# adaly/gridnext

Measured on AMD Instinct MI355X. Metric: spots/sec training throughput (multimodal f+g), higher is better.
Workload: dtype f32; 1 GPU; C4: multimodal f(DenseNet-121 @128px + count-MLP 2000 genes) + hex g on 78x64 Visium grids, 1 array (4992 spots) per GPU per step, f frozen/eval (tutorial mode), g trained with Adam, masked CE; spots_per_array=4992, parallelism=dp1

## Files before the change

### gridnext_amd/_lib.py

```python
import ctypes
import os

import torch

_HERE = os.path.dirname(os.path.abspath(__file__))
LIB_PATH = os.environ.get('GNX_LIB') or os.path.join(_HERE, 'libgridnext_hip.so')

_P, _I, _L, _F, _D = ctypes.c_void_p, ctypes.c_int, ctypes.c_long, ctypes.c_float, ctypes.c_double

SIGNATURES = {
    'gnx_hexconv_fwd': (_I, [_P, _P, _P, _P, _P, _I, _I, _I, _I, _I, _I, _P]),
    'gnx_hexconv_bwd_data': (_I, [_P, _P, _P, _P, _I, _I, _I, _I, _I, _I, _P]),
    'gnx_hexconv_bwd_weight_workspace': (_L, [_I, _I, _I, _I, _I]),
    'gnx_hexconv_bwd_weight': (_I, [_P, _P, _P, _P, _P, _P, _I, _I, _I, _I, _I, _I, _I, _P]),
    'gnx_hexconv_bwd_weight_batch': (_I, [_P, _I, _P]),
    'gnx_bn_workspace': (_L, [_L, _I]),
    'gnx_bn_train_stats': (_I, [_P, _L, _L, _I, _P, _P, _P, _P, _P, _F, _F, _P, _P, _P, _P, _P, _P]),
    'gnx_bn_train_stats_sync': (_I, [_P, _L, _L, _I, _P, _P, _P, _P, _P, _F, _F, _P, _P, _P, _P, _P, _P, _P]),
    'gnx_bn_train_stats_apply': (_I, [_P, _L, _L, _I, _P, _P, _P, _P, _P, _F, _F, _P, _P, _P, _P, _P, _L, _I, _P, _P]),
    'gnx_bn_sync_words': (_L, [_I]),
    'gnx_bn_train_stats_apply_sync': (_I, [_P, _L, _L, _I, _P, _P, _P, _P, _P, _F, _F, _P, _P, _P, _P, _P, _L, _I, _P, _P, _P]),
    'gnx_bn_relu_bwd_sync': (_I, [_P, _L, _P, _L, _P, _L, _L, _I, _P, _P, _P, _P, _P, _P, _I, _I, _I, _I, _P, _P, _P]),
    'gnx_bn_fold_eval': (_I, [_I, _P, _P, _P, _P, _F, _P, _P, _P, _P, _P]),
    'gnx_scale_shift_relu': (_I, [_P, _L, _P, _L, _L, _I, _P, _P, _I, _P]),
# ... 1 lines not shown
    'gnx_bnrelu_avgpool2': (_I, [_P, _L, _P, _L, _L, _I, _I, _P, _P, _P]),
    'gnx_bn_relu_bwd_pooled': (_I, [_P, _L, _P, _L, _P, _L, _L, _I, _I, _P, _P, _P, _P, _P, _P, _I, _P, _P]),
    'gnx_colsum': (_I, [_P, _L, _L, _I, _P, _I, _P, _P]),
    'gnx_masked_ce_workspace': (_L, [_L]),
    'gnx_masked_ce_fwd': (_I, [_P, _L, _P, _L, _I, _I, _F, _P, _P, _P, _P, _P]),
    'gnx_masked_ce_bwd': (_I, [_P, _L, _P, _L, _I, _I, _P, _P, _F, _P, _L, _P]),
    'gnx_meter_add': (_I, [_P, _P, _D, _P, _P, _D, _P]),
    'gnx_conv1x1_bnrelu': (_I, [_P, _L, _P, _P, _L, _L, _I, _I, _P, _P, _I, _I, _P]),
    'gnx_conv1x1_workspace': (_L, [_L, _I, _I]),
    'gnx_conv1x1_bnrelu_ws': (_I, [_P, _L, _P, _P, _L, _L, _I, _I, _P, _P, _P, _P]),
    'gnx_conv1x1_bnrelu_act': (_I, [_P, _L, _P, _P, _L, _L, _I, _I, _P, _P, _P, _P, _P]),
    'gnx_conv1x1_split_pack_halves': (_L, [_I]),
    'gnx_conv1x1_split_pack': (_I, [_P, _P, _I, _P]),
    'gnx_conv1x1_bnrelu_act_split': (_I, [_P, _L, _P, _P, _L, _L, _I, _P, _P, _P, _P, _P]),
    'gnx_conv3x3_split_pack_halves': (_L, []),
    'gnx_conv3x3_split_pack': (_I, [_P, _P, _P]),
    'gnx_conv3x3_split': (_I, [_P, _L, _P, _P, _L, _L, _I, _P]),
    'gnx_wgrad1x1_split_workspace': (_L, [_L, _I, _I]),
    'gnx_wgrad1x1_split': (_I, [_P, _L, _P, _L, _P, _P, _P, _P, _L, _I, _I, _I, _P]),
    'gnx_wgrad3x3_split_workspace': (_L, [_L]),
    'gnx_wgrad3x3_split': (_I, [_P, _L, _P, _L, _P, _P, _L, _I, _I, _P]),
    'gnx_conv1x1_dgrad_bn_workspace': (_L, [_L, _I]),
    'gnx_conv1x1_dgrad_bnrelu_bwd': (_I, [_P, _L, _P, _P, _L, _P, _L, _L, _I, _I, _P, _P, _P, _P, _P, _P, _I, _P, _P]),
    'gnx_conv1x1_dgrad_wgrad_workspace': (_L, [_L, _I]),
    'gnx_conv1x1_dgrad_wgrad_bnrelu_bwd': (_I, [_P, _L, _P, _P, _L, _P, _L, _L, _I, _P, _P, _P, _P, _P, _P, _P, _P, _I, _P]),
    'gnx_conv3x3_dgrad_bn_workspace': (_L, [_L, _I]),
    'gnx_conv3x3_dgrad_bnrelu_bwd': (_I, [_P, _L, _P, _P, _L, _P, _L, _L, _I, _I, _I, _P, _P, _P, _P, _P, _P, _I, _P, _P]),
    'gnx_conv1x1_fold_clamp': (_I, [_P, _P, _P, _P, _P, _P, _P, _P, _I, _I, _P]),
    'gnx_conv1x1_clamped_act': (_I, [_P, _L, _P, _P, _P, _L, _L, _I, _I, _P, _P, _P]),
    'gnx_repack_conv3x3': (_I, [_P, _P, _I, _I, _P]),
    'gnx_conv1x1_bnrelu_f16': (_I, [_P, _L, _P, _P, _L, _L, _I, _I, _P, _P, _I, _I, _P]),
    'gnx_conv3x3_bnrelu_f16': (_I, [_P, _L, _P, _P, _L, _L, _I, _I, _I, _P, _P, _P]),
    'gnx_conv1x1_bnrelu_f16_act16': (_I, [_P, _L, _P, _P, _L, _L, _I, _I, _P, _P, _P, _P, _P]),
    'gnx_conv3x3_f16_dma': (_I, [_P, _L, _P, _P, _L, _L, _I, _I, _I, _P]),
    'gnx_conv_stem_bnrelu_maxpool_h16': (_I, [_P, _P, _P, _L, _L, _I, _I, _I, _I, _I, _I, _I, _I, _P, _P, _P]),
    'gnx_conv_stem_bnrelu_maxpool_u8': (_I, [_P, _P, _P, _L, _L, _I, _I, _I, _I, _I, _I, _I, _I, _P, _P, _P, _I, _P]),
    'gnx_conv_stem_bnrelu_maxpool_f16mul': (_I, [_P, _I, _P, _P, _L, _L, _I, _I, _I, _I, _I, _I, _I, _I, _P, _P, _P, _P]),
    'gnx_u8_to_f32': (_I, [_P, _P, _L, _I, _I, _I, _P, _P]),
    'gnx_conv1x1_bnrelu_f16_h': (_I, [_P, _L, _P, _P, _L, _L, _I, _I, _P, _P, _P, _P, _I, _I, _P]),
    'gnx_conv1x1_bnrelu_h16': (_I, [_P, _L, _P, _P, _L, _L, _I, _I, _P, _P, _P, _P, _P]),
    'gnx_bnrelu_avgpool2_h16': (_I, [_P, _L, _P, _L, _L, _I, _I, _P, _P, _P]),
    'gnx_conv3x3_f16_dma_h': (_I, [_P, _L, _P, _P, _L, _L, _I, _I, _I, _P]),
    'gnx_bnrelu_avgpool_h16': (_I, [_P, _L, _P, _L, _L, _I, _I, _P, _P, _P]),
    'gnx_wgrad1x1_f16_workspace': (_L, [_L, _I, _I]),
    'gnx_wgrad1x1_f16': (_I, [_P, _L, _P, _L, _P, _P, _P, _P, _L, _I, _I, _P, _I, _P, _P]),
    'gnx_wgrad3x3_f16_workspace': (_L, [_L]),
    'gnx_wgrad3x3_f16': (_I, [_P, _L, _P, _P, _P, _L, _I, _P, _I, _P, _P]),
    'gnx_conv3x3_dgrad_bnrelu_bwd_f16_workspace': (_L, [_L]),
    'gnx_conv3x3_dgrad_bnrelu_bwd_f16': (_I, [_P, _L, _P, _P, _P, _L, _I, _P, _P, _P, _P, _P, _P, _P, _I, _P, _P]),
    'gnx_conv1x1_dgrad_bnrelu_bwd_f16_workspace': (_L, [_L, _I]),
    'gnx_conv1x1_dgrad_bnrelu_bwd_f16': (_I, [_P, _P, _P, _L, _P, _L, _L, _I, _P, _P, _P, _P, _P, _P, _P, _P, _I, _P, _P]),
    'gnx_conv1x1_dgrad_wgrad_f16_workspace': (_L, [_L, _I]),
    'gnx_conv1x1_dgrad_wgrad_bnrelu_bwd_f16': (_I, [_P, _P, _P, _L, _P, _L, _L, _I, _P, _P, _P, _P, _P, _P, _P, _P, _P, _I, _P, _P]),
    'gnx_tail_bwd_f16_workspace': (_L, [_L, _I]),
    'gnx_tail_bwd_f16': (_I, [_P, _L, _P, _L, _P, _L, _L, _I, _I, _P, _P, _P, _P, _P, _P, _P, _P, _I, _P, _P]),
    'gnx_trans_bwd_f16_workspace': (_L, [_L, _I, _I]),
    'gnx_trans_bwd_f16': (_I, [_P, _L, _P, _L, _P, _L, _L, _I, _I, _P, _P, _P, _P, _P, _P, _P, _P, _I, _P, _P]),
    'gnx_h16_cols_to_f32': (_I, [_P, _L, _P, _L, _L, _I, _P, _P, _P]),
    'gnx_stem_bwd_f16_workspace': (_L, [_L, _I]),
    'gnx_stem_bwd_f16': (_I, [_P, _P, _P, _P, _P, _P, _P, _L, _P, _P, _P, _P, _L, _I, _I, _P, _I, _P, _P]),
    'gnx_dense_layer_f16_pack': (_I, [_P, _P, _P, _P, _I, _P]),
    'gnx_dense_layer_f16': (_I, [_P, _L, _L, _I, _I, _P, _P, _P, _P, _P, _P, _P]),
    'gnx_dense_layer_f16_tape': (_I, [_P, _L, _L, _I, _I, _P, _P, _P, _P, _P, _P, _P, _L, _P]),
    'gnx_dense_layer_f16_set_form': (_I, [_I]),
    'gnx_dense_bwd_f16_pack': (_I, [_P, _P, _P, _P, _I, _P]),
    'gnx_wgrad3x3_f16_lb': (_I, [_P, _L, _P, _L, _L, _P, _P, _L, _I, _P, _I, _P, _P]),
    'gnx_conv3x3_dgrad_bnrelu_bwd_f16_lb': (_I, [_P, _L, _P, _P, _L, _L, _P, _L, _I, _P, _P, _P, _P, _P, _P, _P, _I, _P, _P]),
    'gnx_conv3x3_bwd_f16_workspace': (_L, [_L]),
    'gnx_conv3x3_bwd_f16_lb': (_I, [_P, _L, _P, _P, _L, _L, _P, _P, _L, _I, _P, _P, _P, _P, _P, _P, _P, _I, _P, _P]),
    'gnx_conv1x1_dgrad_wgrad_bnrelu_bwd_f16_lb': (_I, [_P, _P, _P, _L, _L, _P, _L, _L, _L, _I, _P, _P, _P, _P, _P, _P, _P, _P, _P, _I,
                                                       _P, _P]),
    'gnx_tail_bwd_f16_lb': (_I, [_P, _L, _P, _L, _L, _P, _L, _L, _L, _I, _I, _P, _P, _P, _P, _P, _P, _P, _P, _I, _P, _P]),
    'gnx_trans_bwd_f16_lb': (_I, [_P, _L, _L, _P, _L, _L, _P, _L, _L, _L, _I, _I, _P, _P, _P, _P, _P, _P, _P, _P, _I, _P, _P]),
    'gnx_conv_stem_bnrelu_maxpool_f16mul_cb': (_I, [_P, _I, _P, _P, _L, _L, _I, _I, _I, _I, _I, _I, _I, _I, _P, _P, _P, _P]),
    'gnx_conv1x1_bnrelu_h16_cb': (_I, [_P, _L, _P, _P, _L, _L, _I, _I, _P, _P, _P, _P, _P]),
    'gnx_bnrelu_avgpool2_h16_cb': (_I, [_P, _L, _P, _L, _L, _I, _I, _P, _P, _P]),
    'gnx_transition_f16_pack': (_I, [_P, _P, _I, _I, _P]),
    'gnx_transition_f16': (_I, [_P, _L, _L, _I, _I, _I, _P, _P, _P, _P, _L, _P]),
    'gnx_transition_f16_tape': (_I, [_P, _L, _L, _I, _I, _I, _P, _P, _P, _P, _L, _P, _L, _P]),
    'gnx_bnrelu_avgpool_h16_cb': (_I, [_P, _L, _P, _L, _L, _I, _I, _P, _P, _P]),
    'gnx_conv3x3_bnrelu': (_I, [_P, _L, _P, _P, _L, _L, _I, _I, _I, _P, _P, _P]),
    'gnx_winograd_conv3x3_weights': (_I, [_P, _P, _I, _I, _P]),
    'gnx_conv3x3_winograd': (_I, [_P, _L, _P, _P, _L, _L, _I, _I, _I, _P]),
    'gnx_conv_stem': (_I, [_P, _P, _P, _L, _L, _I, _I, _I, _I, _I, _I, _I, _I, _P]),
    'gnx_conv_stem_bnrelu_maxpool': (_I, [_P, _P, _P, _L, _L, _I, _I, _I, _I, _I, _I, _I, _I, _P, _P, _P]),
    'gnx_conv_stem_bnrelu_maxpool_argmax': (_I, [_P, _P, _P, _L, _P, _L, _I, _I, _I, _I, _I, _I, _I, _I, _P, _P, _P]),
    'gnx_bnrelu_maxpool': (_I, [_P, _L, _P, _L, _L, _I, _I, _I, _P, _P, _P]),
    'gnx_bnrelu_avgpool': (_I, [_P, _L, _P, _L, _L, _I, _I, _P, _P, _P]),
    'gnx_wgrad_workspace': (_L, [_L, _I, _I, _I]),
    'gnx_wgrad_bnrelu': (_I, [_P, _L, _P, _L, _P, _P, _P, _P, _L, _I, _I, _I, _I, _I, _I, _P]),
    'gnx_wgrad_bnrelu_batch': (_I, [_P, _I, _I, _P]),
    'gnx_transpose_weight': (_I, [_P, _P, _I, _I, _P]),
    'gnx_relayout_weights_batch': (_I, [_P, _I, _I, _P]),
    'gnx_repack_conv3x3_bwd': (_I, [_P, _P, _I, _I, _P]),
    'gnx_rows_broadcast': (_I, [_P, _L, _P, _L, _L, _I, _I, _F, _P]),
    'gnx_avgpool2_bwd': (_I, [_P, _L, _P, _L, _L, _I, _I, _P]),
    'gnx_maxpool_bwd': (_I, [_P, _L, _P, _L, _P, _L, _P, _L, _L, _I, _I, _I, _P, _P, _P]),
    'gnx_bnrelu_maxpool_argmax': (_I, [_P, _L, _P, _L, _P, _L, _I, _I, _I, _P, _P, _P]),
    'gnx_maxpool_bwd_argmax': (_I, [_P, _P, _L, _P, _L, _L, _I, _I, _I, _P]),
    'gnx_maxpool_bwd_argmax_bnrelu': (_I, [_P, _P, _L, _P, _L, _P, _P, _L, _L, _I, _I, _I, _P]),
    'gnx_conv0_wgrad_workspace': (_L, [_L, _I, _I, _I, _I, _I, _I, _I]),
    'gnx_conv0_wgrad': (_I, [_P, _P, _L, _P, _P, _L, _I, _I, _I, _I, _I, _I, _I, _I, _P]),
    'gnx_softmax_rows': (_I, [_P, _L, _L, _I, _P, _L, _P, _P]),
    'gnx_gemm_f32': (_I, [_P, _L, _I, _P, _L, _I, _P, _P, _L, _L, _L, _L, _I, _P]),
    'gnx_gemm_f32_workspace': (_L, [_L, _L, _L]),
    'gnx_gemm_f32_ws': (_I, [_P, _L, _I, _P, _L, _I, _P, _P, _L, _L, _L, _L, _I, _P, _P]),
}

_lib = None
_ERRORS = {-1: 'bad argument', -2: 'kernel launch failed', -3: 'unsupported shape'}
ERR_UNSUPPORTED = -3


class HipExtensionMissing(RuntimeError):
    pass


def lib():
    global _lib
    if _lib is None:
        if not os.path.exists(LIB_PATH):
            raise HipExtensionMissing(
                "gridnext_amd: %s not found. Build it with `python -c 'import __graft_entry__ as g; g.build()'` "
                "or `make -C gridnext_amd/csrc`. There is no CPU fallback." % LIB_PATH)
        handle = ctypes.CDLL(LIB_PATH)
        for name, (res, args) in SIGNATURES.items():
            fn = getattr(handle, name)
            fn.restype, fn.argtypes = res, args
        _lib = handle
    return _lib


def stream():
    return torch.cuda.current_stream().cuda_stream


def ptr(t, dtype=torch.float32):
    if t is None:
        return None
    if not t.is_cuda:
        raise RuntimeError("gridnext_amd kernels need tensors on a HIP device (got %s); there is no CPU path"
                           % t.device)
    if dtype is not None and t.dtype != dtype:
        raise TypeError("expected %s, got %s" % (dtype, t.dtype))
    return t.data_ptr()


def call(name, *args):
    rc = getattr(lib(), name)(*args)
    if rc != 0:
        raise RuntimeError("%s failed: %s (%d)" % (name, _ERRORS.get(rc, 'error'), rc))


def try_call(name, *args):
    rc = getattr(lib(), name)(*args)
    if rc == ERR_UNSUPPORTED:
        return False
    if rc != 0:
        raise RuntimeError("%s failed: %s (%d)" % (name, _ERRORS.get(rc, 'error'), rc))
    return True


def query(name, *args):
    return getattr(lib(), name)(*args)
```

### gridnext_amd/csrc/conv3x3.hip

```cpp
#include "fwd_common.h"

namespace {

constexpr int C3_BM = 128, C3_BN = 32;

__global__ __launch_bounds__(256) void conv3x3_kernel(const float* __restrict__ A, long lda,
                                                      const float* __restrict__ Wr, float* __restrict__ out, long ldc,
                                                      long M, int N, int K, int S, const float* __restrict__ scale,
                                                      const float* __restrict__ shift, int vecA, int vecW) {
    extern __shared__ __attribute__((aligned(16))) float lds[];
    const int strip = C3_BM + 2 * S + 2;
    float* As = lds;
    float* Bs = lds + strip * LDK;
    const int t = threadIdx.x, lane = t & 63, wave = t >> 6, h = lane >> 5, i = lane & 31;
    const long P0 = (long)blockIdx.x * C3_BM;
    const long base = P0 - S - 1;
    const int n0 = blockIdx.y * C3_BN;
    const bool has_act = scale != nullptr;

    const long P = P0 + 32 * wave + i;
    unsigned mask = 0;
    if (P < M) {
        const int rem = (int)(P % ((long)S * S));
        const int y = rem / S, x = rem - y * S;
// ... 586 lines not shown
            {
                const char* raw = lds + OFF_RAW + par * RAWB;
#pragma unroll
                for (int j = 0; j < NIT; ++j) {
                    const int it = t + 256 * j;
                    const int c = it / NVR, jp = it - c * NVR;
                    if (it < NVR * 4 && jp < NV) {
                        const int xin = (2 * jp) & (S - 1);
                        auto at = [&](int q) {
                            return raw + (q >> 4) * 1024 + c * 256 + (((q & 15) + ((q >> 4) & 1)) & 15) * 16;
                        };
                        const char* zr = lds + OFF_Z;
                        typedef float f2 __attribute__((ext_vector_type(2)));
                        struct F4 { f2 lo, hi; };
                        auto rd = [&](const char* p) { return *reinterpret_cast<const F4*>(p); };
                        const F4 d0 = rd(xin == 0 ? zr : at(2 * jp)), d1 = rd(at(2 * jp + 1)), d2 = rd(at(2 * jp + 2)),
                                 d3 = rd(xin + 2 == S ? zr : at(2 * jp + 3));
                        char* v = lds + OFF_V + (jp >> 4) * 1024 + c * 256 + (jp & 15) * 16;
                        *reinterpret_cast<F4*>(v) = F4{d0.lo - d2.lo, d0.hi - d2.hi};
                        *reinterpret_cast<F4*>(v + VB) = F4{d1.lo + d2.lo, d1.hi + d2.hi};
                        *reinterpret_cast<F4*>(v + 2 * VB) = F4{d2.lo - d1.lo, d2.hi - d1.hi};
                        *reinterpret_cast<F4*>(v + 3 * VB) = F4{d1.lo - d3.lo, d1.hi - d3.hi};
                    }
                }
            }
#endif
            asm volatile("s_waitcnt lgkmcnt(0)" ::: "memory");
            asm volatile("s_barrier" ::: "memory");
            const unsigned bU = fU + par * UB;
            auto rdA = [&](auto e_c) {
                constexpr int e = decltype(e_c)::value;
                return lds_read4<(e & 1) * 512>(bV[e >> 1]);
            };
            auto rdB = [&](auto e_c) {
                constexpr int e = decltype(e_c)::value;
                return lds_read4<(e >> 1) * 2048 + (e & 1) * 512>(bU);
            };
            f32x4 a = rdA(std::integral_constant<int, 0>{}), bq = rdB(std::integral_constant<int, 0>{});
            static_for<0, 24>([&](auto step_c) {
                constexpr int step = decltype(step_c)::value;
                constexpr int xi = (step >> 1) & 3;
                f32x4 na, nb;
                if constexpr (step < 23) {
                    na = rdA(std::integral_constant<int, step + 1>{});
                    nb = rdB(std::integral_constant<int, step + 1>{});
                    asm volatile("s_waitcnt lgkmcnt(2)" : "+v"(a), "+v"(bq));
                } else {
                    asm volatile("s_waitcnt lgkmcnt(0)" : "+v"(a), "+v"(bq));
                }
                acc[xi][0] = __builtin_amdgcn_mfma_f32_32x32x2f32(a[0], bq[0], acc[xi][0], 0, 0, 0);
                acc[xi][1] = __builtin_amdgcn_mfma_f32_32x32x2f32(a[1], bq[1], acc[xi][1], 0, 0, 0);
                acc[xi][0] = __builtin_amdgcn_mfma_f32_32x32x2f32(a[2], bq[2], acc[xi][0], 0, 0, 0);
                acc[xi][1] = __builtin_amdgcn_mfma_f32_32x32x2f32(a[3], bq[3], acc[xi][1], 0, 0, 0);
#if GNX_WINO_DBG != 2
                if constexpr (step < NSR + NSU) issue_slot(step_c, par ^ 1);
#endif
                if constexpr (step < 23) { a = na; bq = nb; }
            });
            advance_next();
        };
        for (int c2 = 0; c2 < nk2; ++c2) {
            do_chunk(std::integral_constant<int, 0>{});
            do_chunk(std::integral_constant<int, 1>{});
        }
        {
            const int left = M - tile * BM;
            const __amdgpu_buffer_rsrc_t ro = __builtin_amdgcn_make_buffer_rsrc(
                out + (long)tile * BM * ldc, 0, (left < BM ? left : BM) * ldc * 4, 0x00020000);
            const int vo = (2 * (32 * wave + 4 * h) * ldc + i) * 4;
#pragma unroll
            for (int e = 0; e < 16; ++e) {
                const float m0 = acc[0][0][e] + acc[0][1][e], m1 = acc[1][0][e] + acc[1][1][e];
                const float m2 = acc[2][0][e] + acc[2][1][e], m3 = acc[3][0][e] + acc[3][1][e];
                const int row = 2 * ((e & 3) + 8 * (e >> 2));
                __builtin_amdgcn_raw_buffer_store_b32(__float_as_uint((m0 + m1) + m2), ro, vo, row * ldc * 4, 0);
                __builtin_amdgcn_raw_buffer_store_b32(__float_as_uint((m1 - m2) - m3), ro, vo, (row + 1) * ldc * 4, 0);
            }
        }
        stored = true;
    }
    asm volatile("s_waitcnt vmcnt(0)" ::: "memory");
}

__global__ void winograd_weights_kernel(const float* __restrict__ w, float* __restrict__ wu, int N, int K) {
    const long idx = (long)blockIdx.x * blockDim.x + threadIdx.x;
    const long total = (long)3 * N * K;
    if (idx >= total) return;
    const int k = (int)(idx % K), n = (int)((idx / K) % N), dy = (int)(idx / ((long)K * N));
    const float* g = w + ((long)n * K + k) * 9 + dy * 3;
    const float g0 = g[0], g1 = g[1], g2 = g[2];
    const long nk = (long)N * K;
    float* u = wu + (long)dy * 4 * nk + (long)n * K + k;
    u[0] = g0;
    u[nk] = 0.5f * ((g0 + g2) + g1);
    u[2 * nk] = 0.5f * ((g0 + g2) - g1);
    u[3 * nk] = g2;
}

__global__ void repack3x3_kernel(const float* __restrict__ w, float* __restrict__ wr, int N, int K) {
    const long idx = (long)blockIdx.x * blockDim.x + threadIdx.x;
    const long total = (long)9 * N * K;
    if (idx >= total) return;
    const int k = (int)(idx % K), n = (int)((idx / K) % N), tap = (int)(idx / ((long)K * N));
    wr[idx] = w[((long)n * K + k) * 9 + tap];
}

}

GNX_EXPORT int gnx_repack_conv3x3(const float* w, float* wr, int N, int K, hipStream_t stream) {
    if (!w || !wr || N <= 0 || K <= 0) return GNX_ERR_BAD_ARG;
    repack3x3_kernel<<<gnx_cdiv(9L * N * K, 256), 256, 0, stream>>>(w, wr, N, K);
    return gnx_launch_status();
}

GNX_EXPORT int gnx_winograd_conv3x3_weights(const float* w, float* wu, int N, int K, hipStream_t stream) {
    if (!w || !wu || N <= 0 || K <= 0) return GNX_ERR_BAD_ARG;
    winograd_weights_kernel<<<gnx_cdiv(3L * N * K, 256), 256, 0, stream>>>(w, wu, N, K);
    return gnx_launch_status();
}

GNX_EXPORT int gnx_conv3x3_winograd(const float* A, long lda, const float* Wu, float* out, long ldc, long M, int N, int K,
                                    int S, hipStream_t stream) {
    if (!A || !Wu || !out || M < 0 || N <= 0 || K <= 0 || S <= 0 || lda < K || ldc < N || (M % ((long)S * S)) != 0)
        return GNX_ERR_BAD_ARG;
    if (N != 32 || (K & 31) != 0 || !al16(A) || !al16(Wu) || lda % 4 != 0 ||
        M * (lda > ldc ? lda : ldc) >= (1L << 31))
        return GNX_ERR_UNSUPPORTED;
    if (M == 0) return GNX_OK;
    const long wgs = (M + 255) / 256 > 256 ? 256 : (M + 255) / 256;
#define GNX_WINO(SS)                                                                                        \
    conv3x3_wino_kernel<SS><<<(int)wgs, 256, 0, stream>>>(A, (int)lda, Wu, out, (int)ldc, (int)M, K);        \
    return gnx_launch_status()
    switch (S) {
        case 4: GNX_WINO(4);
        case 8: GNX_WINO(8);
        case 16: GNX_WINO(16);
        case 32: GNX_WINO(32);
        case 64: GNX_WINO(64);
        default: return GNX_ERR_UNSUPPORTED;
    }
#undef GNX_WINO
}

GNX_EXPORT long gnx_conv3x3_dgrad_bn_workspace(long M, int N) { return 256L * 8 * 2 * N; }

GNX_EXPORT int gnx_conv3x3_dgrad_bnrelu_bwd(const float* dY, long lddy, const float* Wb, const float* A_act, long lda,
                                            float* dX, long lddx, long M, int N, int K, int S, const float* scale,
                                            const float* shift, const float* mean, const float* invstd, float* dgamma,
                                            float* dbeta, int accumulate, float* workspace, hipStream_t stream) {
    if (!dY || !Wb || !A_act || !dX || !scale || !shift || !mean || !invstd || !workspace || M < 0 || N <= 0 || K <= 0 ||
        S <= 0 || lddy < K || lda < N || lddx < N || (M % ((long)S * S)) != 0)
        return GNX_ERR_BAD_ARG;
    if (K != 32 || N != 128 || (M % C3_BM) != 0 || !al16(dY) || !al16(Wb) || lddy % 4 != 0 ||
        M * (lddy > lddx ? (lddy > lda ? lddy : lda) : (lddx > lda ? lddx : lda)) >= (1L << 31))
        return GNX_ERR_UNSUPPORTED;
    if (M == 0) return GNX_OK;
    C3BnAdj bn = {A_act, (int)lda, scale, shift, mean, invstd, workspace};
    int nblk = 0;
#define GNX_DMAA(SS)                                                                                              \
    do {                                                                                                          \
        if constexpr (SS <= 32) {                                                                                 \
            if (M % 256 == 0 && M / 256 >= 1024) {                                                                \
                nblk = 256 * 8;                                                                                   \
                conv3x3_dma_kernel<SS, 8, 32, true, false, false, true><<<256, 512, 0, stream>>>(                 \
                    dY, (int)lddy, Wb, dX, (int)lddx, (int)M, K, N, bn);                                          \
                break;                                                                                            \
            }                                                                                                     \
        }                                                                                                         \
        const long wgs = M / 128 > 256 ? 256 : M / 128;                                                           \
        nblk = (int)wgs * 4;                                                                                      \
        conv3x3_dma_kernel<SS, 4, 32, true, false, false, true><<<(int)wgs, 256, 0, stream>>>(                    \
            dY, (int)lddy, Wb, dX, (int)lddx, (int)M, K, N, bn);                                                  \
    } while (0)
    switch (S) {
        case 4: GNX_DMAA(4); break;
        case 8: GNX_DMAA(8); break;
        case 16: GNX_DMAA(16); break;
        case 32: GNX_DMAA(32); break;
        case 64: GNX_DMAA(64); break;
        default: return GNX_ERR_UNSUPPORTED;
    }
#undef GNX_DMAA
    if (dgamma || dbeta)
        c3_adj_reduce_kernel<<<gnx_cdiv(2 * N, 64), 64 * C3_ADJ_LANES, 0, stream>>>(workspace, nblk, N, dbeta, dgamma, accumulate);
    return gnx_launch_status();
}

GNX_EXPORT int gnx_conv3x3_bnrelu(const float* A, long lda, const float* Wr, float* out, long ldc, long M, int N, int K,
                                  int S, const float* scale, const float* shift, hipStream_t stream) {
    if (!A || !Wr || !out || M < 0 || N <= 0 || K <= 0 || S <= 0 || lda < K || ldc < N || (!scale) != (!shift) ||
        (M % ((long)S * S)) != 0)
        return GNX_ERR_BAD_ARG;
    if (M == 0) return GNX_OK;
    const size_t lds_bytes = ((size_t)(C3_BM + 2 * S + 2) * LDK + 9 * 32 * LDK + LDK) * sizeof(float);
    if (lds_bytes > 160 * 1024) return GNX_ERR_UNSUPPORTED;
    static size_t configured = 0;
    if (lds_bytes > configured) {
        if (hipFuncSetAttribute(reinterpret_cast<const void*>(conv3x3_kernel), hipFuncAttributeMaxDynamicSharedMemorySize,
                                (int)lds_bytes) != hipSuccess)
            return GNX_ERR_LAUNCH;
        configured = lds_bytes;
    }
    const int vecA = al16(A) && lda % 4 == 0 && K % 4 == 0 && (!scale || (al16(scale) && al16(shift)));
    const int vecW = al16(Wr) && K % 4 == 0;
    dim3 grid(gnx_cdiv(M, C3_BM), gnx_cdiv(N, C3_BN));
    const int nj = gnx_cdiv(C3_BM + 2 * S + 2, 32);
#define GNX_PIPE(NJ)                                                                                              \
    do {                                                                                                          \
        static size_t conf = 0;                                                                                   \
        if (lds_bytes > conf) {                                                                                   \
            if (hipFuncSetAttribute(reinterpret_cast<const void*>(conv3x3_pipe_kernel<NJ>),                       \
                                    hipFuncAttributeMaxDynamicSharedMemorySize, (int)lds_bytes) != hipSuccess)    \
                return GNX_ERR_LAUNCH;                                                                            \
            conf = lds_bytes;                                                                                     \
        }                                                                                                         \
        conv3x3_pipe_kernel<NJ><<<grid, 256, lds_bytes, stream>>>(A, lda, Wr, out, ldc, M, N, K, S, scale, shift, \
                                                                  vecA, vecW);                                    \
    } while (0)
    const bool fast = vecA && vecW;
    if (!scale && fast && N == C3_BN && (K & 63) == 0 && (M % C3_BM) == 0 && M * (lda > ldc ? lda : ldc) < (1L << 31)) {
        const int variant = M / 256 >= 1024 ? 2 : 1;
#define GNX_DMA(SS)                                                                                              \
    do {                                                                                                         \
        if constexpr (SS <= 32) {                                                                                \
// ... 113 lines not shown
```

### include/gridnext_hip.h

```cpp
#ifndef GRIDNEXT_HIP_H
#define GRIDNEXT_HIP_H

#ifdef __cplusplus
extern "C" {
#endif

#define GNX_OK 0
#define GNX_ERR_BAD_ARG (-1)
#define GNX_ERR_LAUNCH (-2)
#define GNX_ERR_UNSUPPORTED (-3)

typedef void* gnx_stream_t;

int gnx_hexconv_fwd(const float* x, const float* kernel0, const float* kernel1, const float* bias, float* y,
                    int B, int H, int W, int I, int O, int mode, gnx_stream_t stream);
int gnx_hexconv_bwd_data(const float* dy, const float* kernel0, const float* kernel1, float* dx,
                         int B, int H, int W, int I, int O, int mode, gnx_stream_t stream);
long gnx_hexconv_bwd_weight_workspace(int B, int H, int W, int I, int O);
int gnx_hexconv_bwd_weight(const float* x, const float* dy, float* dkernel0, float* dkernel1, float* dbias,
                           float* workspace, int B, int H, int W, int I, int O, int mode, int accumulate,
                           gnx_stream_t stream);
typedef struct {
    const float* x; const float* dy; float* dkernel0; float* dkernel1; float* dbias; float* workspace;
    int B, H, W, I, O, mode, accumulate, pad;
// ... 27 lines not shown
                                  float* running_mean, float* running_var, long long* num_batches_tracked, float momentum,
                                  float eps, float* scale, float* shift, float* save_mean, float* save_invstd, float* y, long ldy,
                                  int relu, float* workspace, void* sync, gnx_stream_t stream);
int gnx_bn_relu_bwd_sync(const float* dy, long lddy, const float* x, long ldx, float* dx, long lddx, long M, int C,
                         const float* scale, const float* shift, const float* save_mean, const float* save_invstd, float* dgamma,
                         float* dbeta, int relu, int training, int accumulate, int dx_accumulate, float* workspace, void* sync,
                         gnx_stream_t stream);
int gnx_bnrelu_avgpool2(const float* in, long ldi, float* out, long ldo, long imgs, int C, int S, const float* scale,
                        const float* shift, gnx_stream_t stream);
int gnx_bn_relu_bwd_pooled(const float* dYp, long lddy, const float* x, long ldx, float* dx, long lddx, long imgs, int S,
                           int C, const float* scale, const float* shift, const float* save_mean,
                           const float* save_invstd, float* dgamma, float* dbeta, int accumulate, float* workspace,
                           gnx_stream_t stream);
int gnx_colsum(const float* x, long ld, long M, int C, float* out, int accumulate, float* workspace,
               gnx_stream_t stream);

long gnx_masked_ce_workspace(long M);
int gnx_masked_ce_fwd(const float* logits, long ld, const long long* labels, long M, int C, int label_base,
                      float accum_iters, float* loss, long long* stats, long long* preds, double* workspace,
                      gnx_stream_t stream);
int gnx_masked_ce_bwd(const float* logits, long ld, const long long* labels, long M, int C, int label_base,
                      const long long* stats, const float* dloss, float accum_iters, float* dlogits, long lddz,
                      gnx_stream_t stream);
int gnx_meter_add(double* acc, const float* loss, double weight, const long long* correct, const long long* counted,
                  double counted_const, gnx_stream_t stream);

int gnx_softmax_rows(const float* logits, long ld, long M, int C, float* probs, long ldp, long long* preds,
                     gnx_stream_t stream);

int gnx_gemm_f32(const float* A, long lda, int a_kmajor, const float* B, long ldb, int b_kmajor, const float* bias,
                 float* C, long ldc, long M, long N, long K, int accumulate, gnx_stream_t stream);
long gnx_gemm_f32_workspace(long M, long N, long K);
int gnx_gemm_f32_ws(const float* A, long lda, int a_kmajor, const float* B, long ldb, int b_kmajor, const float* bias,
                    float* C, long ldc, long M, long N, long K, int accumulate, float* workspace, gnx_stream_t stream);

int gnx_conv1x1_bnrelu(const float* A, long lda, const float* W, float* out, long ldc, long M, int N, int K,
                       const float* scale, const float* shift, int pool, int S_in, gnx_stream_t stream);
long gnx_conv1x1_workspace(long M, int N, int K);
int gnx_conv1x1_bnrelu_ws(const float* A, long lda, const float* W, float* out, long ldc, long M, int N, int K,
                          const float* scale, const float* shift, float* workspace, gnx_stream_t stream);
int gnx_conv1x1_bnrelu_act(const float* A, long lda, const float* W, float* out, long ldc, long M, int N, int K,
                           const float* scale, const float* shift, const float* out_scale, const float* out_shift,
                           gnx_stream_t stream);
long gnx_conv1x1_split_pack_halves(int K);
int gnx_conv1x1_split_pack(const float* W, void* Wp, int K, gnx_stream_t stream);
int gnx_conv1x1_bnrelu_act_split(const float* A, long lda, const void* Wp, float* out, long ldc, long M, int K,
                                 const float* scale, const float* shift, const float* out_scale, const float* out_shift,
                                 gnx_stream_t stream);
long gnx_conv3x3_split_pack_halves(void);
int gnx_conv3x3_split_pack(const float* W, void* Wp, gnx_stream_t stream);
int gnx_conv3x3_split(const float* A, long lda, const void* Wp, float* out, long ldc, long M, int S, gnx_stream_t stream);
long gnx_wgrad1x1_split_workspace(long M, int N, int K);
int gnx_wgrad1x1_split(const float* dY, long lddy, const float* X, long ldx, const float* scale, const float* shift, float* dW,
                       float* workspace, long M, int N, int K, int accumulate, gnx_stream_t stream);
long gnx_wgrad3x3_split_workspace(long M);
int gnx_wgrad3x3_split(const float* dY, long lddy, const float* A, long lda, float* dW, float* workspace, long M, int S,
                       int accumulate, gnx_stream_t stream);
long gnx_conv1x1_dgrad_bn_workspace(long M, int N);
int gnx_conv1x1_dgrad_bnrelu_bwd(const float* dY, long lddy, const float* Wt, const float* X, long ldx, float* dX, long lddx,
                                 long M, int N, int K, const float* scale, const float* shift, const float* mean,
                                 const float* invstd, float* dgamma, float* dbeta, int accumulate, float* workspace,
                                 gnx_stream_t stream);
long gnx_conv1x1_dgrad_wgrad_workspace(long M, int K);
int gnx_conv1x1_dgrad_wgrad_bnrelu_bwd(const float* dB, long lddb, const float* W1t, const float* X, long ldx, float* G, long ldg,
                                       long M, int K, const float* scale, const float* shift, const float* mean,
                                       const float* invstd, float* dgamma, float* dbeta, float* dW, float* workspace,
                                       int accumulate, gnx_stream_t stream);
long gnx_conv3x3_dgrad_bn_workspace(long M, int N);
int gnx_conv3x3_dgrad_bnrelu_bwd(const float* dY, long lddy, const float* Wb, const float* A_act, long lda, float* dX,
                                 long lddx, long M, int N, int K, int S, const float* scale, const float* shift,
                                 const float* mean, const float* invstd, float* dgamma, float* dbeta, int accumulate,
                                 float* workspace, gnx_stream_t stream);
int gnx_conv1x1_fold_clamp(const float* W, const float* scale, const float* shift, const float* out_scale,
                           const float* out_shift, float* Wf, float* bounds, float* out_shift_f, int N, int K,
                           gnx_stream_t stream);
int gnx_conv1x1_clamped_act(const float* A, long lda, const float* Wf, const float* bounds, float* out, long ldc, long M,
                            int N, int K, const float* out_scale, const float* out_shift_f, gnx_stream_t stream);
int gnx_repack_conv3x3(const float* w, float* wr, int N, int K, gnx_stream_t stream);
int gnx_conv3x3_bnrelu(const float* A, long lda, const float* Wr, float* out, long ldc, long M, int N, int K, int S,
                       const float* scale, const float* shift, gnx_stream_t stream);
int gnx_winograd_conv3x3_weights(const float* w, float* wu, int N, int K, gnx_stream_t stream);
int gnx_conv3x3_winograd(const float* A, long lda, const float* Wu, float* out, long ldc, long M, int N, int K, int S,
                         gnx_stream_t stream);
int gnx_conv_stem(const float* x, const float* w, float* out, long ldc, long imgs, int Cin, int H, int W, int O,
                  int KH, int KW, int stride, int pad, gnx_stream_t stream);
int gnx_conv_stem_bnrelu_maxpool(const float* x, const float* w, float* out, long ldo, long imgs, int Cin, int H, int W,
                                 int O, int KH, int KW, int stride, int pad, const float* scale, const float* shift,
                                 gnx_stream_t stream);
int gnx_conv_stem_bnrelu_maxpool_argmax(const float* x, const float* w, float* out, long ldo, unsigned char* argmax,
                                        long imgs, int Cin, int H, int W, int O, int KH, int KW, int stride, int pad,
                                        const float* scale, const float* shift, gnx_stream_t stream);
int gnx_bnrelu_maxpool(const float* in, long ldi, float* out, long ldo, long imgs, int C, int Hi, int Wi,
                       const float* scale, const float* shift, gnx_stream_t stream);
int gnx_bnrelu_avgpool(const float* in, long ldi, float* out, long ldo, long imgs, int C, int S2,
                       const float* scale, const float* shift, gnx_stream_t stream);

int gnx_conv1x1_bnrelu_f16(const float* A, long lda, const float* W, float* out, long ldc, long M, int N, int K,
                           const float* scale, const float* shift, int pool, int S_in, gnx_stream_t stream);
int gnx_conv3x3_bnrelu_f16(const float* A, long lda, const float* Wr, float* out, long ldc, long M, int N, int K, int S,
                           const float* scale, const float* shift, gnx_stream_t stream);
int gnx_conv1x1_bnrelu_f16_act16(const float* A, long lda, const float* W, void* out16, long ldc16, long M, int N, int K,
                                 const float* scale, const float* shift, const float* out_scale, const float* out_shift,
                                 gnx_stream_t stream);
int gnx_conv3x3_f16_dma(const void* A16, long lda16, const void* Wr16, float* out, long ldc, long M, int N, int K, int S,
                        gnx_stream_t stream);
int gnx_conv_stem_bnrelu_maxpool_h16(const float* x, const float* w, void* out16, long ldo, long imgs, int Cin, int H, int W,
                                     int O, int KH, int KW, int stride, int pad, const float* scale, const float* shift,
                                     gnx_stream_t stream);
int gnx_conv_stem_bnrelu_maxpool_u8(const unsigned char* x8, const float* w, void* out, long ldo, long imgs, int Cin, int H,
                                    int W, int O, int KH, int KW, int stride, int pad, const float* scale,
                                    const float* shift, const float* norm, int out_f16, gnx_stream_t stream);
int gnx_u8_to_f32(const unsigned char* x8, float* out, long imgs, int C, int H, int W, const float* norm,
                  gnx_stream_t stream);
int gnx_conv_stem_bnrelu_maxpool_f16mul(const void* x, int x_is_u8, const float* w, void* out16, long ldo, long imgs,
                                        int Cin, int H, int W, int O, int KH, int KW, int stride, int pad,
                                        const float* scale, const float* shift, const float* norm, gnx_stream_t stream);
int gnx_conv1x1_bnrelu_f16_h(const void* A16, long lda16, const float* W, void* out16, long ldc16, long M, int N, int K,
                             const float* scale, const float* shift, const float* out_scale, const float* out_shift,
                             int pool, int S_in, gnx_stream_t stream);
int gnx_conv1x1_bnrelu_h16(const void* A16, long lda16, const void* W16, void* out16, long ldc16, long M, int N, int K,
                           const float* scale, const float* shift, const float* out_scale, const float* out_shift,
                           gnx_stream_t stream);
int gnx_bnrelu_avgpool2_h16(const void* in16, long ldi, void* out16, long ldo, long imgs, int C, int S, const float* scale,
                            const float* shift, gnx_stream_t stream);
int gnx_conv3x3_f16_dma_h(const void* A16, long lda16, const void* Wr16, void* out16, long ldc16, long M, int N, int K, int S,
                          gnx_stream_t stream);
int gnx_bnrelu_avgpool_h16(const void* in16, long ldi, float* out, long ldo, long imgs, int C, int S2, const float* scale,
                           const float* shift, gnx_stream_t stream);
int gnx_transition_f16_pack(const float* w, void* wp, int N, int K, hipStream_t stream);
int gnx_transition_f16(const void* X16, long rows_in, long n_img, int S, int K, int N, const void* wp, const float* scale,
                       const float* shift, void* Y16, long rows_out, hipStream_t stream);
int gnx_transition_f16_tape(const void* X16, long rows_in, long n_img, int S, int K, int N, const void* wp, const float* scale,
                            const float* shift, void* Y16, long rows_out, void* P16, long ldp, gnx_stream_t stream);
int gnx_dense_layer_f16_pack(const float* w1, const float* w2, void* w1p, void* w2p, int K, gnx_stream_t stream);
int gnx_dense_layer_f16(void* X16, long rows_total, long n_img, int S, int K, const void* w1p, const void* w2p,
                        const float* scale1, const float* shift1, const float* scale2, const float* shift2, gnx_stream_t stream);
int gnx_dense_layer_f16_tape(void* X16, long rows_total, long n_img, int S, int K, const void* w1p, const void* w2p,
                             const float* scale1, const float* shift1, const float* scale2, const float* shift2, void* A16,
                             long a_rows_total, gnx_stream_t stream);
int gnx_dense_layer_f16_set_form(int form);
int gnx_conv_stem_bnrelu_maxpool_f16mul_cb(const void* x, int x_is_u8, const float* w, void* out16, long rows_total, long imgs,
                                           int Cin, int H, int W, int O, int KH, int KW, int stride, int pad, const float* scale,
                                           const float* shift, const float* norm, gnx_stream_t stream);
int gnx_conv1x1_bnrelu_h16_cb(const void* A16, long lda16, const void* W16, void* out16, long rows_total, long M, int N, int K,
                              const float* scale, const float* shift, const float* out_scale, const float* out_shift,
                              gnx_stream_t stream);
int gnx_bnrelu_avgpool2_h16_cb(const void* in16, long rows_total, void* out16, long ldo, long imgs, int C, int S,
                               const float* scale, const float* shift, gnx_stream_t stream);
int gnx_bnrelu_avgpool_h16_cb(const void* in16, long rows_total, float* out, long ldo, long imgs, int C, int S2,
                              const float* scale, const float* shift, gnx_stream_t stream);

long gnx_wgrad_workspace(long M, int N, int K, int taps);
int gnx_wgrad_bnrelu(const float* dY, long lddy, const float* X, long ldx, const float* scale, const float* shift,
                     float* dW, float* workspace, long M, int N, int K, int S, int taps, int pool, int accumulate,
                     gnx_stream_t stream);
typedef struct {
    const float* dY; long lddy; const float* X; long ldx; const float* scale; const float* shift; float* dW; float* workspace;
    long M; int N, K, S, accumulate;
} gnx_wgrad_item;
int gnx_wgrad_bnrelu_batch(const void* items, int n, int taps, gnx_stream_t stream);
int gnx_transpose_weight(const float* w, float* wt, int N, int K, gnx_stream_t stream);
int gnx_relayout_weights_batch(const void* table, int n, int kind, gnx_stream_t stream);
int gnx_repack_conv3x3_bwd(const float* w, float* wb, int N, int K, gnx_stream_t stream);
int gnx_rows_broadcast(const float* in, long ldi, float* out, long ldo, long imgs, int C, int S2, float alpha,
                       gnx_stream_t stream);
int gnx_avgpool2_bwd(const float* dP, long ldp, float* dA, long lda, long imgs, int C, int S, gnx_stream_t stream);
// ... 77 lines not shown
```

Before: 79550 spots/s.

## Add software-pipelined Winograd conv3x3 kernel overlapping input transform with MFMA

Adds a new Winograd F(2,3) conv3x3 kernel that double-buffers the transformed input tiles and weight chunks in LDS. Raw input loads and the input transform for the next K-chunk are interleaved with the MFMA steps for the current chunk, with hand-tuned waitcnt counts. The default gnx_conv3x3_winograd entry now uses this pipelined kernel, and the old kernel stays reachable through a new serial export. The aim is to hide global-load and transform latency behind matrix math, at the cost of more LDS use, more register pressure and fragile inline-asm synchronisation.

Result: no change. 80270 spots/s (median of 6 runs) (+0.9%).

```diff
diff --git a/gridnext_amd/_lib.py b/gridnext_amd/_lib.py
--- a/gridnext_amd/_lib.py
+++ b/gridnext_amd/_lib.py
@@ -107,6 +107,7 @@
     'gnx_conv3x3_bnrelu': (_I, [_P, _L, _P, _P, _L, _L, _I, _I, _I, _P, _P, _P]),
     'gnx_winograd_conv3x3_weights': (_I, [_P, _P, _I, _I, _P]),
     'gnx_conv3x3_winograd': (_I, [_P, _L, _P, _P, _L, _L, _I, _I, _I, _P]),
+    'gnx_conv3x3_winograd_serial': (_I, [_P, _L, _P, _P, _L, _L, _I, _I, _I, _P]),
     'gnx_conv_stem': (_I, [_P, _P, _P, _L, _L, _I, _I, _I, _I, _I, _I, _I, _I, _P]),
     'gnx_conv_stem_bnrelu_maxpool': (_I, [_P, _P, _P, _L, _L, _I, _I, _I, _I, _I, _I, _I, _I, _P, _P, _P]),
     'gnx_conv_stem_bnrelu_maxpool_argmax': (_I, [_P, _P, _P, _L, _P, _L, _I, _I, _I, _I, _I, _I, _I, _I, _P, _P, _P]),
diff --git a/gridnext_amd/csrc/conv3x3.hip b/gridnext_amd/csrc/conv3x3.hip
--- a/gridnext_amd/csrc/conv3x3.hip
+++ b/gridnext_amd/csrc/conv3x3.hip
@@ -692,6 +692,232 @@
     asm volatile("s_waitcnt vmcnt(0)" ::: "memory");
 }
 
+__device__ __forceinline__ f32x4 buf_load4(const __amdgpu_buffer_rsrc_t& r, unsigned voff, int soff) {
+    f32x4 v;
+    asm volatile("buffer_load_dwordx4 %0, %1, %2, %3 offen" : "=v"(v) : "v"(voff), "s"(r), "s"(soff));
+    return v;
+}
+template <int OFF>
+__device__ __forceinline__ void lds_write4(unsigned addr, f32x4 v) {
+    asm volatile("ds_write_b128 %0, %1 offset:%2" ::"v"(addr), "v"(v), "n"(OFF) : "memory");
+}
+__device__ __forceinline__ float sub_f32(float a, float b) {
+    float r;
+    asm volatile("v_sub_f32 %0, %1, %2" : "=v"(r) : "v"(a), "v"(b));
+    return r;
+}
+__device__ __forceinline__ float add_f32(float a, float b) {
+    float r;
+    asm volatile("v_add_f32 %0, %1, %2" : "=v"(r) : "v"(a), "v"(b));
+    return r;
+}
+template <int N>
+__device__ __forceinline__ void vm_wait() {
+    asm volatile("s_waitcnt vmcnt(%0)" ::"n"(N) : "memory");
+}
+
+template <int S>
+__global__ __launch_bounds__(256) void conv3x3_wino_pipe_kernel(const float* __restrict__ A, int lda,
+                                                               const float* __restrict__ Wu, float* __restrict__ out,
+                                                               int ldc, int M, int K) {
+    constexpr int BM = 256, NPAIR = 128;
+    constexpr int NV = NPAIR + S;
+    constexpr int NIT = 3, NVP = 64 * NIT;
+    static_assert(4 * NV <= 256 * NIT, "items");
+    constexpr int UB = 12 * 32 * 64, VB = NVP * 64, VD = 4 * VB + 1024;
+    constexpr int OFF_U = 0, OFF_V = 2 * UB, LDSB = OFF_V + 2 * VD;
+    static_assert(LDSB <= 160 * 1024, "LDS");
+    constexpr int NSU = 6;
+    constexpr unsigned OOB = 0x80000000u;
+    __shared__ __attribute__((aligned(16))) char lds[LDSB];
+    const int t = threadIdx.x, lane = t & 63, h = lane >> 5, i = lane & 31;
+    reinterpret_cast<float*>(lds + OFF_V + 4 * VB)[t] = 0.f;
+    reinterpret_cast<float*>(lds + OFF_V + VD + 4 * VB)[t] = 0.f;
+    const int T = (M + BM - 1) / BM;
+    const int nch = K >> 4;
+    int G = gridDim.x;
+    asm volatile("" : "+s"(G));
+    asm volatile("" : "+s"(M), "+s"(lda));
+    const int bx = blockIdx.x;
+    const int bid = (G & 7) == 0 ? (bx & 7) * (G >> 3) + (bx >> 3) : bx;
+    auto tile_of = [&](int round) {
+        const int base = round * G;
+        return base + (base + G <= T ? bid : bx);
+    };
+    const unsigned lb = lds_addr(lds);
+    const int wave = __builtin_amdgcn_readfirstlane(t >> 6);
+
+    const unsigned voffU = ((unsigned)(lane & 15) * K + 4 * (lane >> 4)) * 4u;
+    const __amdgpu_buffer_rsrc_t rU = __builtin_amdgcn_make_buffer_rsrc(const_cast<float*>(Wu), 0, 12 * 32 * K * 4, 0x00020000);
+    int uchunk = 0;
+    auto issue_u = [&](auto slot_c, auto buf_c) {
+        constexpr int slot = decltype(slot_c)::value, buf = decltype(buf_c)::value;
+        const int p = wave + 4 * slot;
+        dma16_buf(rU, voffU, (16 * p * K + 16 * uchunk) * 4, lds_addr(lds + OFF_U + buf * UB + p * 1024));
+    };
+
+    int rround = 0, rtile = tile_of(0), rchunk = 0;
+    __amdgpu_buffer_rsrc_t rs;
+    unsigned rsh = 0;
+    auto set_raw_tile = [&]() {
+        const int rowbase = rtile * BM - S - 1;
+        const int lo = rowbase < 0 ? 0 : rowbase;
+        const int hi = rowbase + 2 * NVP + 2 < M ? rowbase + 2 * NVP + 2 : M;
+        rs = __builtin_amdgcn_make_buffer_rsrc(const_cast<float*>(A + (long)lo * lda), 0, (unsigned)(hi - lo) * lda * 4u,
+                                               0x00020000);
+        rsh = (unsigned)(lo - rowbase) * lda * 4u;
+    };
+    set_raw_tile();
+    auto advance_raw = [&]() {
+        if (++rchunk == nch) {
+            rchunk = 0;
+            rtile = tile_of(++rround);
+            if (rtile >= T) rtile = bid;
+            set_raw_tile();
+        }
+    };
+    unsigned voff[NIT][4], vw[2][NIT];
+#pragma unroll
+    for (int j = 0; j < NIT; ++j) {
+        const int it = t + 256 * j;
+        const int jp = (it & 7) | ((it >> 5) << 3), c = (it >> 3) & 3;
+        const int xin = (2 * jp) & (S - 1);
+#pragma unroll
+        for (int k = 0; k < 4; ++k) voff[j][k] = (unsigned)(2 * jp + k) * lda * 4u + 16u * c;
+        if (xin == 0) voff[j][0] = OOB;
+        if (xin + 2 == S) voff[j][3] = OOB;
+        vw[0][j] = lb + OFF_V + (jp >> 4) * 1024 + c * 256 + (jp & 15) * 16;
+        vw[1][j] = vw[0][j] + VD;
+    }
+    f32x4 rd[NIT][4];
+    auto load_item = [&](auto j_c) {
+        constexpr int j = decltype(j_c)::value;
+        const int soff = 64 * rchunk;
+        if (rsh) {
+#pragma unroll
+            for (int k = 0; k < 4; ++k) rd[j][k] = buf_load4(rs, voff[j][k] == OOB ? OOB : voff[j][k] - rsh, soff);
+        } else {
+#pragma unroll
+            for (int k = 0; k < 4; ++k) rd[j][k] = buf_load4(rs, voff[j][k], soff);
+        }
+    };
+    f32x4 vt;
+    auto xform = [&](auto j_c, auto ph_c, auto dbuf_c) {
+        constexpr int j = decltype(j_c)::value, ph = decltype(ph_c)::value, dbuf = decltype(dbuf_c)::value;
+        constexpr int xi = ph >> 1, e = 2 * (ph & 1);
+        const f32x4 &d0 = rd[j][0], &d1 = rd[j][1], &d2 = rd[j][2], &d3 = rd[j][3];
+        if constexpr (ph == 2 || ph == 4 || ph == 6) lds_write4<(xi - 1) * VB>(vw[dbuf][j], vt);
+#pragma unroll
+        for (int q = e; q < e + 2; ++q) {
+            if constexpr (xi == 0) vt[q] = sub_f32(d0[q], d2[q]);
+            else if constexpr (xi == 1) vt[q] = add_f32(d1[q], d2[q]);
+            else if constexpr (xi == 2) vt[q] = sub_f32(d2[q], d1[q]);
+            else vt[q] = sub_f32(d1[q], d3[q]);
+        }
+        if constexpr (ph == 7) lds_write4<3 * VB>(vw[dbuf][j], vt);
+    };
+
+    static_for<0, NSU>([&](auto sc) { issue_u(sc, std::integral_constant<int, 0>{}); });
+    uchunk = 1 % nch;
+    static_for<0, NIT>([&](auto jc) { load_item(jc); });
+    advance_raw();
+    static_for<0, NIT>([&](auto jc) {
+        vm_wait<0>();
+        static_for<0, 8>([&](auto ph) { xform(jc, ph, std::integral_constant<int, 0>{}); });
+    });
+    static_for<0, NIT>([&](auto jc) { load_item(jc); });
+    advance_raw();
+
+    const int r = 32 * wave + i;
+    const unsigned bU = lb + OFF_U + (i >> 4) * 1024 + (i & 15) * 16 + h * 256;
+
+    bool stored = false;
+    for (int round = 0, tile = tile_of(0); tile < T; tile = tile_of(++round)) {
+        const int P = tile * BM + 2 * r;
+        const int y = (P % (S * S)) / S;
+        unsigned bV[12];
+#pragma unroll
+        for (int dy = 0; dy < 3; ++dy) {
+            const int jp = r + S / 2 + (dy - 1) * (S / 2);
+            const bool ok = (dy == 1) || (dy == 0 ? y > 0 : y < S - 1);
+#pragma unroll
+            for (int xi = 0; xi < 4; ++xi)
+                bV[dy * 4 + xi] = ok ? lb + OFF_V + xi * VB + (jp >> 4) * 1024 + (jp & 15) * 16 + h * 256 : lb + OFF_V + 4 * VB;
+        }
+        f32x16 acc[4][2];
+#pragma unroll
+        for (int xi = 0; xi < 4; ++xi)
+#pragma unroll
+            for (int q = 0; q < 2; ++q)
+#pragma unroll
+                for (int e = 0; e < 16; ++e) acc[xi][q][e] = 0.f;
+
+        auto do_chunk = [&](auto par_c, bool st) {
+            constexpr int par = decltype(par_c)::value;
+            if (st) asm volatile("s_waitcnt vmcnt(44) lgkmcnt(0)" ::: "memory");
+            else asm volatile("s_waitcnt vmcnt(12) lgkmcnt(0)" ::: "memory");
+            asm volatile("s_barrier" ::: "memory");
+            auto rdA = [&](auto e_c) {
+                constexpr int e = decltype(e_c)::value;
+                return lds_read4<(e & 1) * 512 + par * VD>(bV[e >> 1]);
+            };
+            auto rdB = [&](auto e_c) {
+                constexpr int e = decltype(e_c)::value;
+                return lds_read4<(e >> 1) * 2048 + (e & 1) * 512 + par * UB>(bU);
+            };
+            f32x4 a = rdA(std::integral_constant<int, 0>{}), bq = rdB(std::integral_constant<int, 0>{});
+            static_for<0, 24>([&](auto step_c) {
+                constexpr int step = decltype(step_c)::value;
+                constexpr int xi = (step >> 1) & 3;
+                constexpr int j = step >> 3, ph = step & 7;
+                f32x4 na, nb;
+                if constexpr (step < 23) {
+                    na = rdA(std::integral_constant<int, step + 1>{});
+                    nb = rdB(std::integral_constant<int, step + 1>{});
+                    asm volatile("s_waitcnt lgkmcnt(2)" : "+v"(a), "+v"(bq));
+                } else {
+                    asm volatile("s_waitcnt lgkmcnt(0)" : "+v"(a), "+v"(bq));
+                }
+                acc[xi][0] = __builtin_amdgcn_mfma_f32_32x32x2f32(a[0], bq[0], acc[xi][0], 0, 0, 0);
+                acc[xi][1] = __builtin_amdgcn_mfma_f32_32x32x2f32(a[1], bq[1], acc[xi][1], 0, 0, 0);
+                acc[xi][0] = __builtin_amdgcn_mfma_f32_32x32x2f32(a[2], bq[2], acc[xi][0], 0, 0, 0);
+                acc[xi][1] = __builtin_amdgcn_mfma_f32_32x32x2f32(a[3], bq[3], acc[xi][1], 0, 0, 0);
+                if constexpr (ph == 0) {
+                    if (st) vm_wait<(j == 0 ? 8 : 14) + 32>();
+                    else vm_wait<(j == 0 ? 8 : 14)>();
+                }
+                if constexpr (step < NSU) issue_u(step_c, std::integral_constant<int, par ^ 1>{});
+                xform(std::integral_constant<int, j>{}, std::integral_constant<int, ph>{}, std::integral_constant<int, par ^ 1>{});
+                if constexpr (ph == 7) load_item(std::integral_constant<int, j>{});
+                if constexpr (step < 23) { a = na; bq = nb; }
+            });
+            uchunk = uchunk + 1 == nch ? 0 : uchunk + 1;
+            advance_raw();
+        };
+        for (int c2 = 0; c2 < nch / 2; ++c2) {
+            do_chunk(std::integral_constant<int, 0>{}, stored);
+            stored = false;
+            do_chunk(std::integral_constant<int, 1>{}, false);
+        }
+        {
+            const int left = M - tile * BM;
+            const __amdgpu_buffer_rsrc_t ro = __builtin_amdgcn_make_buffer_rsrc(
+                out + (long)tile * BM * ldc, 0, (left < BM ? left : BM) * ldc * 4, 0x00020000);
+            const int vo = (2 * (32 * wave + 4 * h) * ldc + i) * 4;
+#pragma unroll
+            for (int e = 0; e < 16; ++e) {
+                const float m0 = acc[0][0][e] + acc[0][1][e], m1 = acc[1][0][e] + acc[1][1][e];
+                const float m2 = acc[2][0][e] + acc[2][1][e], m3 = acc[3][0][e] + acc[3][1][e];
+                const int row = 2 * ((e & 3) + 8 * (e >> 2));
+                __builtin_amdgcn_raw_buffer_store_b32(__float_as_uint((m0 + m1) + m2), ro, vo, row * ldc * 4, 0);
+                __builtin_amdgcn_raw_buffer_store_b32(__float_as_uint((m1 - m2) - m3), ro, vo, (row + 1) * ldc * 4, 0);
+            }
+        }
+        stored = true;
+    }
+    asm volatile("s_waitcnt vmcnt(0)" ::: "memory");
+}
+
 __global__ void winograd_weights_kernel(const float* __restrict__ w, float* __restrict__ wu, int N, int K) {
     const long idx = (long)blockIdx.x * blockDim.x + threadIdx.x;
     const long total = (long)3 * N * K;
@@ -729,8 +955,9 @@
     return gnx_launch_status();
 }
 
-GNX_EXPORT int gnx_conv3x3_winograd(const float* A, long lda, const float* Wu, float* out, long ldc, long M, int N, int K,
-                                    int S, hipStream_t stream) {
+template <bool PIPE>
+static int conv3x3_winograd_launch(const float* A, long lda, const float* Wu, float* out, long ldc, long M, int N, int K,
+                                   int S, hipStream_t stream) {
     if (!A || !Wu || !out || M < 0 || N <= 0 || K <= 0 || S <= 0 || lda < K || ldc < N || (M % ((long)S * S)) != 0)
         return GNX_ERR_BAD_ARG;
     if (N != 32 || (K & 31) != 0 || !al16(A) || !al16(Wu) || lda % 4 != 0 ||
@@ -738,8 +965,10 @@
         return GNX_ERR_UNSUPPORTED;
     if (M == 0) return GNX_OK;
     const long wgs = (M + 255) / 256 > 256 ? 256 : (M + 255) / 256;
-#define GNX_WINO(SS)                                                                                        \
-    conv3x3_wino_kernel<SS><<<(int)wgs, 256, 0, stream>>>(A, (int)lda, Wu, out, (int)ldc, (int)M, K);        \
+    const bool pipe = PIPE && lda < (1L << 20);
+#define GNX_WINO(SS)                                                                                            \
+    if (pipe) conv3x3_wino_pipe_kernel<SS><<<(int)wgs, 256, 0, stream>>>(A, (int)lda, Wu, out, (int)ldc, (int)M, K); \
+    else conv3x3_wino_kernel<SS><<<(int)wgs, 256, 0, stream>>>(A, (int)lda, Wu, out, (int)ldc, (int)M, K);       \
     return gnx_launch_status()
     switch (S) {
         case 4: GNX_WINO(4);
@@ -750,6 +979,15 @@
         default: return GNX_ERR_UNSUPPORTED;
     }
 #undef GNX_WINO
+}
+
+GNX_EXPORT int gnx_conv3x3_winograd(const float* A, long lda, const float* Wu, float* out, long ldc, long M, int N, int K,
+                                    int S, hipStream_t stream) {
+    return conv3x3_winograd_launch<true>(A, lda, Wu, out, ldc, M, N, K, S, stream);
+}
+GNX_EXPORT int gnx_conv3x3_winograd_serial(const float* A, long lda, const float* Wu, float* out, long ldc, long M, int N,
+                                           int K, int S, hipStream_t stream) {
+    return conv3x3_winograd_launch<false>(A, lda, Wu, out, ldc, M, N, K, S, stream);
 }
 
 GNX_EXPORT long gnx_conv3x3_dgrad_bn_workspace(long M, int N) { return 256L * 8 * 2 * N; }
diff --git a/include/gridnext_hip.h b/include/gridnext_hip.h
--- a/include/gridnext_hip.h
+++ b/include/gridnext_hip.h
@@ -133,6 +133,8 @@
 int gnx_winograd_conv3x3_weights(const float* w, float* wu, int N, int K, gnx_stream_t stream);
 int gnx_conv3x3_winograd(const float* A, long lda, const float* Wu, float* out, long ldc, long M, int N, int K, int S,
                          gnx_stream_t stream);
+int gnx_conv3x3_winograd_serial(const float* A, long lda, const float* Wu, float* out, long ldc, long M, int N, int K, int S,
+                                gnx_stream_t stream);
 int gnx_conv_stem(const float* x, const float* w, float* out, long ldc, long imgs, int Cin, int H, int W, int O,
                   int KH, int KW, int stride, int pad, gnx_stream_t stream);
 int gnx_conv_stem_bnrelu_maxpool(const float* x, const float* w, float* out, long ldo, long imgs, int Cin, int H, int W,
```
